# adolliou/euispice_coreg

Measured on AMD Instinct MI355X. Metric: lag-points/sec (whole node) on 2048² grid, 60×60 CRVAL sweep; argmax-shift match, higher is better.
Workload: dtype f64; 1 GPU; headline: Carrington 'fa' 2048x2048 grid lon(200,300) lat(-20,20), 60x60 CRVAL lags arange(-30,30,1) arcsec, small 2048^2 HRIEUV-like, ref 3072^2 FSI-like, order 2, solar_r 1.004; lag_points=3600, parallelism=single GPU, no collective, resident=True, sweeps_in_flight=2, small_stored_f32=True, use_lds=True

## Files before the change

euispice_coreg_amd/csrc/coreg_hip.hip:

```cpp
#include <hip/hip_runtime.h>

#include <algorithm>
#include <chrono>
#include <cmath>
#include <cstdio>
#include <cstdlib>
#include <cstring>
#include <limits>
#include <condition_variable>
#include <map>
#include <memory>
#include <mutex>
#include <string>
#include <thread>
#include <functional>
#include <type_traits>
#include <utility>
#include <vector>

#include "fit.hpp"
#include "geometry.hpp"
#include "kernels.hpp"
#include <atomic>
#include "ricecomp.hpp"
// ... 14 lines not shown
#include "host_sweep_launch.hpp"
#include "host_sweep_mi.hpp"
#include "host_fix_lists.hpp"
#include "host_sweep_io.hpp"
#include "host_context.hpp"
#include "pixels_plan.hpp"
#include "host_pixels.hpp"

coreg_handle::~coreg_handle() = default;

extern "C" {

const char* coreg_version(void) { return "coreg_hip " COREG_VERSION " (gfx950)"; }

int coreg_create(coreg_handle** out, int device) {
    if (!out) return COREG_EINVAL;
    *out = nullptr;
    int ndev = 0;
    hipError_t e = hipGetDeviceCount(&ndev);
    if (e != hipSuccess || ndev < 1) return COREG_EHIP;
    if (device < 0) {
        if (hipGetDevice(&device) != hipSuccess) device = 0;
    }
    if (device >= ndev) return COREG_EINVAL;
    coreg_handle* h = new (std::nothrow) coreg_handle();
    if (!h) return COREG_ENOMEM;
    h->device = device;
    if (hipSetDevice(device) != hipSuccess || hipStreamCreateWithFlags(&h->stream.s, hipStreamNonBlocking) != hipSuccess ||
        hipEventCreate(&h->ev_end[0].e) != hipSuccess ||
        hipEventCreate(&h->ev_end[1].e) != hipSuccess || hipEventRecord(h->ev_end[0], h->stream) != hipSuccess ||
        hipEventRecord(h->ev_end[1], h->stream) != hipSuccess ||
        h->pivots.reserve(2 * sizeof(double)) != hipSuccess ||
        hipMemsetAsync(h->pivots.p, 0, 2 * sizeof(double), h->stream) != hipSuccess) {
        coreg_destroy(h);
        return COREG_EHIP;
    }
    std::memset(&h->stats, 0, sizeof(h->stats));
    *out = h;
    return COREG_OK;
}

void coreg_destroy(coreg_handle* h) {
    if (!h) return;
    (void)hipSetDevice(h->device);
    if (h->up_thread.joinable()) {
        {
            std::unique_lock<std::mutex> lk(h->up_m);
            h->up_cv.wait(lk, [&] { return !h->up_busy && !h->up_has; });
            h->up_stop = true;
        }
        h->up_cv.notify_all();
        h->up_thread.join();
    }
    if (h->stream) (void)hipStreamSynchronize(h->stream);
    if (h->up_stream) (void)hipStreamSynchronize(h->up_stream);
    delete h;
}

const char* coreg_last_error(const coreg_handle* h) { return h ? h->err.c_str() : "null handle"; }

int coreg_set_stream(coreg_handle* h, void* hip_stream) {
    if (!h) return COREG_EINVAL;
    RETCHK(bind_device(h));
    RETCHK(collect_stats(h));
    HIPCHK(hipStreamSynchronize(h->stream));
    HIPCHK(h->stream.borrow((hipStream_t)hip_stream));
    return COREG_OK;
}

int coreg_synchronize(coreg_handle* h) {
    if (!h) return COREG_EINVAL;
    RETCHK(bind_device(h));
    HIPCHK(hipStreamSynchronize(h->stream));
    return COREG_OK;
}

int coreg_set_option(coreg_handle* h, const char* name, int64_t value) {
    if (!h || !name) return COREG_EINVAL;
    const std::string n(name);
    if (n == "use_lds") {
        h->opt_use_lds = value ? 1 : 0;
    } else if (n == "clean_path") {
        h->opt_clean_path = value ? 1 : 0;
    } else if (n == "tap_nan_filter") {
        if (value < 0 || value > 2) return fail(h, COREG_EINVAL, "tap_nan_filter must be 0, 1 or 2");
        h->opt_tap_nan_filter = value;
    } else if (n == "overlap_upload") {
        h->opt_overlap_upload = value ? 1 : 0;
    } else if (n == "async_upload") {
        h->opt_async_upload = value ? 1 : 0;
    } else if (n == "refine") {
        h->opt_refine = value ? 1 : 0;
    } else if (n == "refine_cond_log10") {
        if (value < -3 || value > 15) return fail(h, COREG_EINVAL, "refine_cond_log10 must be in [-3, 15]");
        h->opt_refine_cond_log10 = value;
    } else if (n == "refine_max") {
        if (value < 0 || value > 16) return fail(h, COREG_EINVAL, "refine_max must be in [0, 16]");
    } else if (n == "tile_w") {
        if (value != 0 && (value < 1 || value > kTilePts || (value & (value - 1)) != 0))
            return fail(h, COREG_EINVAL, "tile_w must be 0 or a power of two <= 1024");
        h->opt_tile_w = value;
    } else if (n == "n_groups") {
        if (value < 0) return fail(h, COREG_EINVAL, "n_groups must be >= 0");
        h->opt_n_groups = value;
    } else if (n == "sweep_wgs") {
        if (value < 0) return fail(h, COREG_EINVAL, "sweep_wgs must be >= 0");
        h->opt_sweep_wgs = value;
    } else if (n == "skew") {
        (void)value;
    } else if (n == "shard_world") {
        if (value < 1 || value > 64) return fail(h, COREG_EINVAL, "shard_world must be in [1, 64]");
        h->opt_shard_world = value;
        if (h->opt_shard_rank >= value) h->opt_shard_rank = 0;
    } else if (n == "combo_begin") {
        if (value < 0) return fail(h, COREG_EINVAL, "combo_begin must be >= 0");
        h->opt_combo_begin = value;
    } else if (n == "combo_end") {
        if (value < 0) return fail(h, COREG_EINVAL, "combo_end must be >= 0");
        h->opt_combo_end = value;
    } else if (n == "shard_rank") {
        if (value < 0 || value >= h->opt_shard_world) return fail(h, COREG_EINVAL, "shard_rank must be in [0, shard_world)");
        h->opt_shard_rank = value;
    } else if (n == "border_fix") {
        h->opt_border_fix = value ? 1 : 0;
    } else if (n == "tap_fix") {
        h->opt_tap_fix = value ? 1 : 0;
    } else if (n == "tap_cap") {
        if (value < 1 || value > (1 << 26)) return fail(h, COREG_EINVAL, "tap_cap must be in [1, 2^26]");
        h->opt_tap_cap = value;
    } else if (n == "pitch") {
        h->opt_pitch = value;
    } else if (n == "taper_frac") {
        if (value < -1 || value > 1000) return fail(h, COREG_EINVAL, "taper_frac must be in [-1, 1000]");
        h->opt_taper_frac = value;
    } else if (n == "taper_min") {
        if (value < 16 || value > 1024) return fail(h, COREG_EINVAL, "taper_min must be in [16, 1024]");
        h->opt_taper_min = value;
    } else if (n == "taper_rounds") {
        if (value < 1) return fail(h, COREG_EINVAL, "taper_rounds must be >= 1");
        h->opt_taper_rounds = value;
    } else if (n == "crop_reference") {
        h->opt_crop_reference = value ? 1 : 0;
    } else if (n == "tile_skip") {
        h->opt_tile_skip = value ? 1 : 0;
    } else if (n == "h_series") {
        h->opt_h_series = value ? 1 : 0;
    } else if (n == "h_incr") {
        h->opt_h_incr = value ? 1 : 0;
    } else if (n == "patch_w") {
        if (value < 0 || value > kBlock) return fail(h, COREG_EINVAL, "patch_w must be in [0, 256]");
        h->opt_patch_w = value;
    } else if (n == "mi_chunks") {
        if (value < 0 || value > kMiMaxChunks) return fail(h, COREG_EINVAL, "mi_chunks must be in [0, 64]");
        h->opt_mi_chunks = value;
    } else if (n == "lds_bytes") {
        if (value < 1024 || value > 159 * 1024) return fail(h, COREG_EINVAL, "lds_bytes must be in [1 KiB, 159 KiB]");
        h->opt_lds_bytes = value;
    } else {
        return fail(h, COREG_EINVAL, "unknown option: " + n);
    }
    return COREG_OK;
}

}

#include "abi_images.hpp"
// ... 8 lines not shown
```

euispice_coreg_amd/csrc/host_state.hpp:

```cpp
#pragma once
namespace {

enum SrcKind {
    SRC_HOST = 0,
    SRC_PINNED = 1,
    SRC_DEVICE = 2,
    SRC_TILED = 3,
};

struct PixFmt {
    int bitpix = 0;
    bool f32 = false;
    double bscale = 1.0, bzero = 0.0;
    bool raw() const { return bitpix != 0; }
    bool scaled() const { return bscale != 1.0 || bzero != 0.0; }
    size_t elem() const { return raw() ? (size_t)(bitpix < 0 ? -bitpix : bitpix) / 8 : (f32 ? 4 : 8); }
    bool swap_only() const { return bitpix == -32 && !scaled(); }
    static PixFmt native(bool is_f32) {
        PixFmt f;
        f.f32 = is_f32;
        return f;
    }
};

// ... 45 lines not shown
    int gW = 0, gH = 0;
    int ref_dtype = -1;
    DevBuf pivots, red_sum, red_cnt;
    DevBuf t_sin_lon, t_cos_lon, t_cos_lat, t_sin_lat, t_lon_deg, t_dx;
    coreg_diffrot rot_ref = {}, rot_small = {};
    bool has_rot_ref = false, has_rot_small = false;
    CarrTables tabs;
    std::vector<double> tabs_key;
    bool tabs_uploaded = false;
    PinBuf pin_img[2];
    Event ev_img[2];
    int pin_img_next = 0;
    DevBuf pts, tile_count, tile_list, tile_cum, group_first, tile_info, tile_bbox;
    DevBuf visit_rec;
    DevBuf rf_fix_slab;
    DevBuf counters;
    DevBuf lane_params, out_index, partials, out_dev, tmp_img;
    DevBuf sweep_queue;
    int n_cus = 0;
    struct SweepResidency {
        const void* fn;
        size_t lds_bytes;
        int per_cu;
    };
    std::vector<SweepResidency> sweep_residency;
    int64_t opt_sweep_wgs = 0;
    DevBuf counts;
    long long counts_n = -1;
    DevBuf up_f64, up_flag;
    DevBuf up_raw;
    DevBuf rice_blob, rice_rand, dec_img;
    PrologueArgs pending_prologue = {};
    DevBuf bbox_buf;
    Stream aux_stream;
    Stream up_stream;
    Event ev_small, ev_main;
    bool small_pending = false;
    DevBuf red_sum_up, red_cnt_up;
    int64_t opt_overlap_upload = 1;
    int64_t opt_tap_nan_filter = 2;
    int64_t opt_async_upload = 0;
    std::thread up_thread;
    std::mutex up_m;
    std::condition_variable up_cv;
    std::function<hipError_t()> up_job;
    bool up_has = false, up_stop = false, up_busy = false;
    hipError_t up_rc = hipSuccess;
    PinBuf pin_small[2];
    Event ev_pin_small[2];
    int pin_small_next = 0;
    WcslibCaches wcslib;
    DevBuf border_flags, fix_partial;
    DevBuf border_dev;
    PinBuf pin_border;
    int64_t opt_border_fix = 1;
    int64_t opt_tap_fix = 1, opt_tap_cap = 1 << 24;
    DevBuf tap_count, tap_segq, tap_list, tap_skip, tap_seg_slot, tap_seg_begin, tap_pixel, tap_xw, tap_yw;
    long long tap_last[3] = {0, 0, 0};
    int last_variant[7] = {-1, 0, 0, 0, 0, 0, 0};
    int64_t opt_shard_world = 1, opt_shard_rank = 0;
    int64_t opt_combo_begin = 0, opt_combo_end = 0;
    DevBuf sums;
    long long sums_slots = 0;
    struct PendingFinalize {
        long long slot_off, n_slots, lag_begin;
        int residus;
        RefineArgs refine;
        std::function<int(coreg_handle*)> replay_precompute;
        FixLaunch fixes;
    };
    std::function<int(coreg_handle*)> last_precompute;
    PlanMemo plan_memo;
    DevBuf rf_flags, rf_pivots, rf_list, rf_head, rf_partial;
    std::vector<PendingFinalize> pending_fin;
    DevBuf fin_outidx;
    long long pending_n_out = 0;
    std::vector<double> mi_edges_small, mi_edges_large;
    DevBuf mi_hist;
    size_t mi_lds[6] = {0, 0, 0, 0, 0, 0};
    int64_t opt_mi_chunks = 0;

    int64_t opt_crop_reference = 1;
    int64_t opt_taper_min = 128, opt_taper_frac = -1, opt_taper_rounds = 6;
    int64_t opt_use_lds = 1, opt_clean_path = 1, opt_refine = 1, opt_refine_cond_log10 = 5, opt_tile_w = 0, opt_n_groups = 0, opt_lds_bytes = (159 * 1024 * kPointGroups) / 4, opt_patch_w = 0, opt_h_series = 1, opt_h_incr = 1, opt_tile_skip = 1, opt_pitch = -1;

    coreg_stats stats;
    bool stats_pending = false;
    PinBuf pin_info;
    std::vector<EventPair> ev_sweep, ev_pre;
    size_t ev_sweep_used = 0, ev_pre_used = 0;
    hipEvent_t ev_t1 = nullptr;
    Event ev_end[2];
    PinBuf pin_plan[2];
    int plan_slot = 0;
    bool plan_open = false;
};
```

euispice_coreg_amd/csrc/host_sweep_launch.hpp:

```cpp
#pragma once
namespace {
using sweep_variant::SweepVariant;
static_assert(sweep_variant::kTranslate == MODE_TRANSLATE && sweep_variant::kHomography == MODE_HOMOGRAPHY &&
                  sweep_variant::kHomographySeries == MODE_HOMOGRAPHY_SERIES && sweep_variant::kCar == MODE_CAR &&
                  sweep_variant::kOrderRt == ORDER_RT, "sweep_variant.hpp restates the kernels' constants");

struct SweepLaunchSpec {
    int mode = MODE_TRANSLATE;
    int order = 2;
    int method = COREG_METHOD_CORRELATION;
    size_t slot_off = 0;
    int n_batches = 0, n_tiles = 0;
    long long lag_begin = 0;
    double* out_dev = nullptr;
    const LaunchU* car_inv = nullptr;
    const BorderFix* fix = nullptr;
    int pitch_sel = 0;
    long long n_slots() const { return (long long)n_batches * kBlock; }
    bool residus() const { return method != COREG_METHOD_CORRELATION; }
    int residus_kind() const { return method == COREG_METHOD_RESIDUS_MASKED ? 2 : (residus() ? 1 : 0); }
    const double* params_dev(const coreg_handle* h) const {
        return h->lane_params.as<double>() + (mode == MODE_TRANSLATE ? 2 : 9) * slot_off;
    }
    const long long* outidx_dev(const coreg_handle* h) const { return h->out_index.as<long long>() + slot_off; }
// ... 6 lines not shown
template <size_t... I>
SweepKernel* sweep_kernel_table(std::index_sequence<I...>) {
    constexpr const SweepVariant* v = sweep_variant::kSweepVariants.v;
    static SweepKernel table[] = {
        {k_sweep<v[I].mode, v[I].order, std::conditional_t<v[I].f32, float, double>, v[I].round, v[I].resid, v[I].pitch>, {0}}...};
    return table;
}

int raise_dynamic_lds(coreg_handle* h, SweepKernel* k, size_t lds_bytes) {
    std::lock_guard<std::mutex> lock(g_attr_mutex);
    size_t& ab = k->attr_bytes[h->device % kMaxDevices];
    if (lds_bytes > 48 * 1024 && lds_bytes > ab) {
        HIPCHK(hipFuncSetAttribute((const void*)k->fn, hipFuncAttributeMaxDynamicSharedMemorySize, (int)lds_bytes));
        ab = lds_bytes;
    }
    return COREG_OK;
}

int sweep_grid(coreg_handle* h, const SweepKernel* k, size_t lds_bytes, long long items, unsigned* grid) {
    long long resident = h->opt_sweep_wgs;
    if (resident <= 0) {
        if (h->n_cus <= 0) HIPCHK(hipDeviceGetAttribute(&h->n_cus, hipDeviceAttributeMultiprocessorCount, h->device));
        int per_cu = 0;
        for (const coreg_handle::SweepResidency& r : h->sweep_residency)
            if (r.fn == (const void*)k->fn && r.lds_bytes == lds_bytes) per_cu = r.per_cu;
        if (per_cu <= 0) {
            HIPCHK(hipOccupancyMaxActiveBlocksPerMultiprocessor(&per_cu, (const void*)k->fn, kSweepThreads, lds_bytes));
            if (per_cu <= 0) return fail(h, COREG_EHIP, "launch_sweep: the device holds no k_sweep workgroup of this LDS size");
            h->sweep_residency.push_back({(const void*)k->fn, lds_bytes, per_cu});
        }
        resident = (long long)h->n_cus * per_cu;
    }
    *grid = (unsigned)(8 * ((std::min(items, resident) + 7) / 8));
    return COREG_OK;
}

int launch_k_sweep(coreg_handle* h, const SweepLaunchSpec& L, SweepArgs a, int n_groups8, size_t lds_bytes) {
    const SweepVariant v = sweep_variant::pick_sweep_variant(L.mode, L.order, h->small_f32, L.residus(), L.pitch_sel);
    const int at = sweep_variant::sweep_variant_index(v);
    if (at < 0) return fail(h, COREG_EINVAL, "launch_sweep: no k_sweep instantiation for this mode / order / pitch");
    SweepKernel* k = sweep_kernel_table(std::make_index_sequence<sweep_variant::kNumSweepVariants>()) + at;
    EventPair* ev = next_event(h, h->ev_sweep, h->ev_sweep_used);
    if (!ev) return fail(h, COREG_EHIP, "hipEventCreate failed");
    RETCHK(raise_dynamic_lds(h, k, lds_bytes));
    a.items8 = n_groups8 * L.n_batches;
    unsigned grid = 0;
    RETCHK(sweep_grid(h, k, lds_bytes, 8LL * a.items8, &grid));
    HIPCHK(h->sweep_queue.reserve(8 * sizeof(unsigned)));
    a.queue = h->sweep_queue.as<unsigned>();
    HIPCHK(hipMemsetAsync(a.queue, 0, 8 * sizeof(unsigned), h->stream));
    HIPCHK(hipEventRecord(ev->a, h->stream));
    hipLaunchKernelGGL(k->fn, dim3(grid), dim3(kSweepThreads), lds_bytes, h->stream, a);
    HIPCHK(hipEventRecord(ev->b, h->stream));
    HIPCHK(hipGetLastError());
    const int rec[7] = {at, v.mode, v.order, v.f32 ? 1 : 0, v.round ? 1 : 0, v.resid ? 1 : 0, v.pitch};
    std::copy(rec, rec + 7, h->last_variant);
    return COREG_OK;
}

SweepArgs sweep_args(const coreg_handle* h, const SweepLaunchSpec& L, int n_groups, int group_lo, size_t lds_bytes) {
    SweepArgs a;
    a.img = h->small.p;
    a.W = h->sW;
    a.H = h->sH;
    a.pts = h->pts.as<Pt>();
    a.tile_count = h->tile_count.as<int>();
    a.tile_list = h->tile_list.as<int>();
    a.tile_cum = h->tile_cum.as<int>();
    a.group_first = h->group_first.as<int>();
    a.tile_info = h->tile_info.as<long long>();
    a.tile_bbox = h->tile_bbox.as<double>();
    a.visit_rec = h->visit_rec.as<VisitRec>();
    a.lane_params = L.params_dev(h);
    a.n_slots = L.n_slots();
    a.n_batches = L.n_batches;
    a.n_groups = n_groups;
    a.group_lo = group_lo;
    a.partials = h->partials.as<double>();
    a.queue = nullptr;
    a.items8 = 0;
    a.pivots = h->pivots.as<double>();
    a.use_lds = h->opt_use_lds ? 1 : 0;
    a.clean_path = h->opt_clean_path ? 1 : 0;
    a.lds_elems = (int)(lds_bytes / sizeof(double));
    a.car_inv = L.car_inv ? *L.car_inv : LaunchU{};
    a.car_inv.order_rt = L.order;
    a.car_inv.h_incr = (int)h->opt_h_incr;
    return a;
}

template <typename Args>
void fill_fix_common(Args& x, const coreg_handle* h, const SweepLaunchSpec& L) {
    x.img = h->small.p;
    x.W = h->sW;
    x.H = h->sH;
    x.ref = h->ref.p;
    x.ref_f32 = h->ref_dtype == COREG_F32 ? 1 : 0;
    x.gw = h->gW;
    x.order = L.order;
    x.round_f32 = L.mode == MODE_TRANSLATE ? 0 : 1;
    x.residus = L.residus() ? 1 : 0;
    x.pivots = h->pivots.as<double>();
    x.hom = L.params_dev(h);
    x.n_slots = L.n_slots();
}

int build_fix_launch(coreg_handle* h, const SweepLaunchSpec& L, FixLaunch* fl) {
    fl->small_f32 = h->small_f32;
    if (!L.fix || !L.fix->any()) return COREG_OK;
    static const std::vector<BorderItems::Item> no_items;
    for (const BorderItems::Item& it : L.fix->border ? L.fix->border->items : no_items) {
        if (it.flags_off >= 0) {
            ParityFixArgs p = {};
            fill_fix_common(p, h, L);
            p.flags = h->border_flags.as<unsigned char>() + it.flags_off;
            p.gh = h->gH;
            p.slot = it.slot;
            p.n_partial = 256;
            if (h->fix_partial.reserve((size_t)p.n_partial * kNumSums * sizeof(double)) != hipSuccess)
                return fail(h, COREG_EHIP, "hipMalloc failed (parity fix)");
            p.partial = h->fix_partial.as<double>();
            fl->parity.push_back(p);
        }
        if (it.n == 0) continue;
        BorderFixArgs b = {};
        fill_fix_common(b, h, L);
        b.slot = it.slot;
        b.dropped = h->border_dev.as<int>() + it.first;
        b.n_dropped = it.n;
        fl->border.push_back(b);
    }
    if (L.fix->tap.segs > 0) {
        fl->tap = L.fix->tap;
        fill_fix_common(fl->tap.args, h, L);
    }
    return COREG_OK;
}

int keep_tap_lists(coreg_handle* h, FixLaunch* fixes) {
    auto kept = std::make_shared<KeptTapLists>();
    const size_t nseg = (size_t)fixes->tap.segs, cnt = (size_t)fixes->tap.count;
    TapFixArgs& t = fixes->tap.args;
    const void* src[5] = {t.xw, t.yw, t.pixel, t.seg_begin, t.seg_slot};
    const size_t bytes[5] = {cnt * sizeof(double), cnt * sizeof(double), cnt * sizeof(unsigned), (nseg + 1) * sizeof(int),
                             nseg * sizeof(int)};
    size_t off[6] = {0};
    for (int k = 0; k < 5; ++k) off[k + 1] = off[k] + ((bytes[k] + 7) & ~(size_t)7);
    HIPCHK(kept->all.reserve(off[5]));
    char* all = kept->all.as<char>();
    for (int k = 0; k < 5; ++k)
        if (bytes[k]) HIPCHK(hipMemcpyAsync(all + off[k], src[k], bytes[k], hipMemcpyDeviceToDevice, h->stream));
    t.xw = (const double*)(all + off[0]);
    t.yw = (const double*)(all + off[1]);
    t.pixel = (const unsigned*)(all + off[2]);
    t.seg_begin = (const int*)(all + off[3]);
    t.seg_slot = (const int*)(all + off[4]);
    fixes->kept = kept;
    return COREG_OK;
}

int queue_pending_finalize(coreg_handle* h, const SweepLaunchSpec& L, const RefineArgs& refine, bool refinable,
                           const FixLaunch& fl) {
    coreg_handle::PendingFinalize pf;
    pf.slot_off = (long long)L.slot_off;
    pf.n_slots = L.n_slots();
    pf.lag_begin = L.lag_begin;
// ... 73 lines not shown
```

euispice_coreg_amd/csrc/kernels_sweep.hpp:

```cpp
#pragma once
namespace coreg {
struct SweepArgs {
    const void* img;
    int W, H;
    const Pt* pts;
    const int* tile_count;
    const int* tile_list;
    const int* tile_cum;
    const int* group_first;
    long long* tile_info;
    const double* tile_bbox;
    const VisitRec* visit_rec;
    const double* lane_params;
    long long n_slots;
    int n_batches;
    int n_groups;
    int group_lo;
    double* partials;
    unsigned* queue;
    int items8;
    const double* pivots;
    int use_lds;
    int clean_path;
    int lds_elems;
    LaunchU car_inv;
};

struct Acc {
    int n;
    double a, b, aa, bb, ab;
};

template <int N>
struct Taps;
template <>
struct Taps<3> {
    double t[9];
    __device__ __forceinline__ void issue(unsigned a0, unsigned a1, unsigned a2) {
        asm volatile(
            "ds_read_b64 %0, %9\n\tds_read_b64 %1, %9 offset:8\n\tds_read_b64 %2, %9 offset:16\n\t"
            "ds_read_b64 %3, %10\n\tds_read_b64 %4, %10 offset:8\n\tds_read_b64 %5, %10 offset:16\n\t"
            "ds_read_b64 %6, %11\n\tds_read_b64 %7, %11 offset:8\n\tds_read_b64 %8, %11 offset:16"
            : "=&v"(t[0]), "=&v"(t[1]), "=&v"(t[2]), "=&v"(t[3]), "=&v"(t[4]), "=&v"(t[5]), "=&v"(t[6]), "=&v"(t[7]),
              "=&v"(t[8])
            : "v"(a0), "v"(a1), "v"(a2));
    }
    __device__ __forceinline__ void wait_after(double& w0, double& w1, double& w2) {
        asm volatile("s_waitcnt lgkmcnt(0)"
                     : "+v"(t[0]), "+v"(t[1]), "+v"(t[2]), "+v"(t[3]), "+v"(t[4]), "+v"(t[5]), "+v"(t[6]), "+v"(t[7]),
                       "+v"(t[8]), "+v"(w0), "+v"(w1), "+v"(w2));
    }
    __device__ __forceinline__ void issue_before(unsigned a0, unsigned a1, unsigned a2, double& fx, double& fy) {
        asm volatile(
            "ds_read_b64 %0, %11\n\tds_read_b64 %1, %11 offset:8\n\tds_read_b64 %2, %11 offset:16\n\t"
            "ds_read_b64 %3, %12\n\tds_read_b64 %4, %12 offset:8\n\tds_read_b64 %5, %12 offset:16\n\t"
            "ds_read_b64 %6, %13\n\tds_read_b64 %7, %13 offset:8\n\tds_read_b64 %8, %13 offset:16"
            : "=&v"(t[0]), "=&v"(t[1]), "=&v"(t[2]), "=&v"(t[3]), "=&v"(t[4]), "=&v"(t[5]), "=&v"(t[6]), "=&v"(t[7]),
              "=&v"(t[8]), "+v"(fx), "+v"(fy)
            : "v"(a0), "v"(a1), "v"(a2));
    }
    __device__ __forceinline__ void wait() {
        asm volatile("s_waitcnt lgkmcnt(0)"
                     : "+v"(t[0]), "+v"(t[1]), "+v"(t[2]), "+v"(t[3]), "+v"(t[4]), "+v"(t[5]), "+v"(t[6]), "+v"(t[7]),
                       "+v"(t[8]));
    }
    template <int P>
    __device__ __forceinline__ void issue_before_imm(unsigned a0, double& fx, double& fy) {
        static_assert(P > 0 && (2 * P + 2) * 8 < 65536, "LDS immediate offsets are 16 bits");
        asm volatile(
            "ds_read_b64 %0, %11\n\tds_read_b64 %1, %11 offset:8\n\tds_read_b64 %2, %11 offset:16\n\t"
            "ds_read_b64 %3, %11 offset:%12\n\tds_read_b64 %4, %11 offset:%13\n\tds_read_b64 %5, %11 offset:%14\n\t"
            "ds_read_b64 %6, %11 offset:%15\n\tds_read_b64 %7, %11 offset:%16\n\tds_read_b64 %8, %11 offset:%17"
            : "=&v"(t[0]), "=&v"(t[1]), "=&v"(t[2]), "=&v"(t[3]), "=&v"(t[4]), "=&v"(t[5]), "=&v"(t[6]), "=&v"(t[7]),
              "=&v"(t[8]), "+v"(fx), "+v"(fy)
            : "v"(a0), "n"(P * 8), "n"(P * 8 + 8), "n"(P * 8 + 16), "n"(2 * P * 8), "n"(2 * P * 8 + 8),
              "n"(2 * P * 8 + 16));
    }
};
template <>
struct Taps<2> {
    double t[4];
    __device__ __forceinline__ void issue(unsigned a0, unsigned a1, unsigned) {
        asm volatile(
            "ds_read_b64 %0, %4\n\tds_read_b64 %1, %4 offset:8\n\t"
            "ds_read_b64 %2, %5\n\tds_read_b64 %3, %5 offset:8"
            : "=&v"(t[0]), "=&v"(t[1]), "=&v"(t[2]), "=&v"(t[3])
            : "v"(a0), "v"(a1));
    }
    __device__ __forceinline__ void issue_before(unsigned a0, unsigned a1, unsigned a2, double&, double&) {
        issue(a0, a1, a2);
    }
    __device__ __forceinline__ void wait() {
        asm volatile("s_waitcnt lgkmcnt(0)" : "+v"(t[0]), "+v"(t[1]), "+v"(t[2]), "+v"(t[3]));
    }
};

template <>
struct Taps<4> {
    double t[16];
    __device__ __forceinline__ void issue_before(unsigned a0, unsigned a1, unsigned a2, unsigned a3, double& fx,
                                                 double& fy) {
        asm volatile(
            "ds_read_b64 %0, %18\n\tds_read_b64 %1, %18 offset:8\n\tds_read_b64 %2, %18 offset:16\n\t"
            "ds_read_b64 %3, %18 offset:24\n\t"
            "ds_read_b64 %4, %19\n\tds_read_b64 %5, %19 offset:8\n\tds_read_b64 %6, %19 offset:16\n\t"
            "ds_read_b64 %7, %19 offset:24\n\t"
// ... 449 lines not shown
                            ux = xn * r;
                            uy = yn * r;
                        }
                        point_lag<MODE, ORDER, TS, LDS, ROUND, RESID, INTERIOR, PITCH, CLEAN, true>(
                            acc, win, img, pitch, ox, oy, W, H, wmax, hmax, px0, py0, pxw, pyw, hv, cu, ux, uy,
                            spt_f64(cur, 2), spt_f64(cur, 3), pivot_b);
                        if constexpr (CLEAN) {
                            if (k == 1) acc.a += spt_f64(cur, 3);
                            if (k == 2) acc.aa += spt_f64(cur, 3);
                            if (k == kChunk - 1) acc.n += kChunk;
                        }
                        spt_wait(nxt);
                        cur = nxt;
                    }
                }
            }
            if (pg == n_full % kPointGroups) {
                for (int p = n_full * kChunk; p < p_end; ++p) {
                    Pt pt;
                    load_pt_uniform(pts + p, pt);
                    point_lag<MODE, ORDER, TS, LDS, ROUND, RESID, INTERIOR, PITCH>(acc, win, img, pitch, ox, oy, W, H, wmax,
                                                                                   hmax, px0, py0, pxw, pyw, hm, cu, pt.b0,
                                                                                   pt.b1, pt.a, pt.pad, pivot_b);
                }
            }
            return;
        }
    }
    {
        int c = p_begin / kChunk + pg;
        if (c < n_full) {
            H9 hml = hm;
            double& anchor = MODE == MODE_TRANSLATE ? (INTERIOR && LDS ? pxw : px0) : hml.h[MODE == MODE_CAR ? 0 : 7];
            SPt cur = spt_load(pts + c * kChunk, anchor);
            spt_wait(cur);
            for (; c < n_full; c += kPointGroups) {
                const Pt* __restrict__ q = pts + c * kChunk;
#pragma unroll
                for (int k = 0; k < kChunk; ++k) {
                    SPt nxt = spt_load(k + 1 < kChunk ? q + k + 1 : q + kPointGroups * kChunk, anchor);
                    point_lag<MODE, ORDER, TS, LDS, ROUND, RESID, INTERIOR, PITCH, CLEAN>(
                        acc, win, img, pitch, ox, oy, W, H, wmax, hmax, px0, py0, pxw, pyw, hml, cu, spt_f64(cur, 0),
                        spt_f64(cur, 1), spt_f64(cur, 2), spt_f64(cur, 3), pivot_b);
                    if constexpr (CLEAN) {
                        if (k == 1) acc.a += spt_f64(cur, 3);
                        if (k == 2) acc.aa += spt_f64(cur, 3);
                        if (k == kChunk - 1) acc.n += kChunk;
                    }
                    spt_wait(nxt);
                    cur = nxt;
                }
            }
        }
    }
#else
    for (int c = p_begin / kChunk + pg; c < n_full; c += kPointGroups) {
        const Pt* __restrict__ q = pts + c * kChunk;
        Pt pt[kChunk];
#pragma unroll
        for (int k = 0; k < kChunk; ++k) load_pt_uniform(q + k, pt[k]);
#pragma unroll
        for (int k = 0; k < kChunk; ++k)
            point_lag<MODE, ORDER, TS, LDS, ROUND, RESID, INTERIOR, PITCH, CLEAN>(acc, win, img, pitch, ox, oy, W, H, wmax,
                                                                                  hmax, px0, py0, pxw, pyw, hm, cu, pt[k].b0,
                                                                                  pt[k].b1, pt[k].a, pt[k].pad, pivot_b);
        if constexpr (CLEAN) {
            acc.n += kChunk;
            acc.a += pt[1].pad;
            acc.aa += pt[2].pad;
        }
    }
#endif
    if (pg == n_full % kPointGroups) {
        for (int p = n_full * kChunk; p < p_end; ++p) {
            Pt pt;
            load_pt_uniform(pts + p, pt);
            point_lag<MODE, ORDER, TS, LDS, ROUND, RESID, INTERIOR, PITCH>(acc, win, img, pitch, ox, oy, W, H, wmax, hmax,
                                                                           px0, py0, pxw, pyw, hm, cu, pt.b0, pt.b1, pt.a,
                                                                           pt.pad, pivot_b);
        }
    }
}

template <int MODE, int ORDER, typename TS, bool ROUND, bool RESID, int PITCH = 0>
__global__ void __launch_bounds__(kSweepThreads) k_sweep(const SweepArgs a) {
    extern __shared__ __align__(16) unsigned char lds_raw[];
    double* lds = (double*)lds_raw;
    constexpr int kWaves = kSweepThreads / 64;
    constexpr int kLagWaves = kBlock / 64;
    __shared__ double wred2[2][kLagWaves][4];
    __shared__ int wdirty[2][kWaves];
    constexpr bool kCleanPath = MODE != MODE_CAR && !RESID && ORDER != ORDER_RT && !(ROUND && sizeof(TS) == 8);
    int n_vis = 0, n_vis_lds = 0, n_vis_int = 0, n_vis_clean = 0;

    __shared__ int next_q[2];
    const int slot8 = blockIdx.x & 7;
    int q = blockIdx.x >> 3;
    int item_par = 0;

    const int lane = threadIdx.x & 63, wave = threadIdx.x >> 6;
    const int pg = __builtin_amdgcn_readfirstlane(wave % kPointGroups);
    const int lw = __builtin_amdgcn_readfirstlane(wave / kPointGroups);
    const int ls = 64 * lw + lane;

    const TS* __restrict__ img = (const TS*)a.img;
    const int W = a.W, H = a.H;
    const double inf = __builtin_inf();
    const double pivot_b = a.pivots[1];
#if defined(__HIP_DEVICE_COMPILE__)
    const unsigned win = (unsigned)(uintptr_t)(__attribute__((address_space(3))) unsigned char*)lds_raw;
#else
    const unsigned win = 0;
#endif

    while (q < a.items8) {
    const int batch = q % a.n_batches;
    const int group = a.group_lo + (q / a.n_batches) * 8 + slot8;
    const long long slot = (long long)batch * kBlock + ls;
    int visit = 0;

    double px0 = 0.0, py0 = 0.0;
    H9 hm;
#pragma unroll
    for (int k = 0; k < 9; ++k) hm.h[k] = 0.0;
    if (MODE == MODE_TRANSLATE) {
        px0 = a.lane_params[slot];
        py0 = a.lane_params[a.n_slots + slot];
    } else {
#pragma unroll
        for (int k = 0; k < 9; ++k) hm.h[k] = a.lane_params[(long long)k * a.n_slots + slot];
    }

    const bool pad_lane = MODE == MODE_TRANSLATE ? (px0 != px0) : (hm.h[8] != hm.h[8]);

    Acc acc = {0, 0.0, 0.0, 0.0, 0.0, 0.0};

    const int u_lo = a.group_first[1024 + group];
    const int u_hi = a.group_first[1024 + group + 1];

    constexpr bool kLagBox = MODE == MODE_TRANSLATE && COREG_VISIT_LAGBOX;
    double lx0 = 0.0, lx1 = 0.0, ly0 = 0.0, ly1 = 0.0;
    if constexpr (kLagBox) {
        lx0 = lx1 = px0;
        ly0 = ly1 = py0;
        for (int o = 32; o > 0; o >>= 1) {
            lx0 = fmin(lx0, __shfl_xor(lx0, o));
            lx1 = fmax(lx1, __shfl_xor(lx1, o));
            ly0 = fmin(ly0, __shfl_xor(ly0, o));
            ly1 = fmax(ly1, __shfl_xor(ly1, o));
        }
        if (lane == 0 && pg == 0) {
            wred2[0][lw][0] = lx0;
            wred2[0][lw][1] = lx1;
            wred2[0][lw][2] = ly0;
            wred2[0][lw][3] = ly1;
        }
        __syncthreads();
        lx0 = fmin(fmin(wred2[0][0][0], wred2[0][1][0]), fmin(wred2[0][2][0], wred2[0][3][0]));
        lx1 = fmax(fmax(wred2[0][0][1], wred2[0][1][1]), fmax(wred2[0][2][1], wred2[0][3][1]));
        ly0 = fmin(fmin(wred2[0][0][2], wred2[0][1][2]), fmin(wred2[0][2][2], wred2[0][3][2]));
        ly1 = fmax(fmax(wred2[0][0][3], wred2[0][1][3]), fmax(wred2[0][2][3], wred2[0][3][3]));
    }

    int tl = a.group_first[group];
    unsigned park = 0;
    {
        Visit first;
        load_visit_uniform(a.visit_rec + tl, first);
        park = park_visit(first, park);
    }
    for (; u_lo < u_hi; ++tl) {
        Visit cur;
        unpark_visit(park, cur);
        const int ubase = cur.ubase;
        if (ubase >= u_hi) break;
        Visit nxt;
        load_visit_uniform(a.visit_rec + tl + 1, nxt);
        const int tile = cur.tile;
        const int cnt = cur.cnt;
        const int p_begin = max(u_lo - ubase, 0) * kUnitPts;
        const int p_end = min((u_hi - ubase) * kUnitPts, cnt);
        if (p_begin >= p_end) {
            park = park_visit(nxt, park);
            continue;
        }
        const double bx0 = cur.bx0, bx1 = cur.bx1, by0 = cur.by0, by1 = cur.by1;

        double mnx, mxx, mny, mxy;
        if constexpr (kLagBox) {
            mnx = bx0 + lx0;
            mxx = bx1 + lx1;
            mny = by0 + ly0;
            mxy = by1 + ly1;
        } else if (MODE == MODE_TRANSLATE) {
            mnx = bx0 + px0;
            mxx = bx1 + px0;
            mny = by0 + py0;
            mxy = by1 + py0;
        } else {
            mnx = inf; mxx = -inf; mny = inf; mxy = -inf;
#pragma unroll
            for (int c = 0; c < 4; ++c) {
                double cx, cy;
                apply_map<MODE>(hm, a.car_inv, (c & 1) ? bx1 : bx0, (c & 2) ? by1 : by0, cx, cy);
                mnx = fmin(mnx, cx);
                mxx = fmax(mxx, cx);
                mny = fmin(mny, cy);
                mxy = fmax(mxy, cy);
            }
            if (MODE == MODE_CAR) {
                const double margin = car_tile_margin(a.car_inv.box_c, fmax(fabs(by0), fabs(by1)) + a.car_inv.pole_sep);
                mnx -= margin;
                mxx += margin;
                mny -= margin;
                mxy += margin;
            }
        }
        int* wdirt = wdirty[visit & 1];
        if constexpr (!kLagBox) {
            for (int o = 32; o > 0; o >>= 1) {
                mnx = fmin(mnx, __shfl_xor(mnx, o));
                mxx = fmax(mxx, __shfl_xor(mxx, o));
                mny = fmin(mny, __shfl_xor(mny, o));
                mxy = fmax(mxy, __shfl_xor(mxy, o));
            }
            double(*wred)[4] = wred2[visit & 1];
            if (lane == 0 && pg == 0) {
                wred[lw][0] = mnx;
                wred[lw][1] = mxx;
                wred[lw][2] = mny;
                wred[lw][3] = mxy;
            }
            __syncthreads();
            mnx = fmin(fmin(wred[0][0], wred[1][0]), fmin(wred[2][0], wred[3][0]));
            mxx = fmax(fmax(wred[0][1], wred[1][1]), fmax(wred[2][1], wred[3][1]));
            mny = fmin(fmin(wred[0][2], wred[1][2]), fmin(wred[2][2], wred[3][2]));
            mxy = fmax(fmax(wred[0][3], wred[1][3]), fmax(wred[2][3], wred[3][3]));
        }
        ++visit;
        if (!(mxx >= 0.0) || !(mnx <= (double)(W - 1)) || !(mxy >= 0.0) || !(mny <= (double)(H - 1))) {
            park = park_visit(nxt, park);
            continue;
        }
        if constexpr (kLagBox) __syncthreads();
        constexpr double kClear = 1e-9;
        const bool interior = (mnx >= kClear) & (mxx <= (double)(W - 1) - kClear) & (mny >= kClear) &
                              (mxy <= (double)(H - 1) - kClear);
        constexpr bool kWide = ORDER == ORDER_RT || ORDER > 2;
        const int ord = ORDER == ORDER_RT ? a.car_inv.order_rt : ORDER;
        const int ap_lo = kWide ? ord / 2 + 1 : 1;
        const int ap_hi = kWide ? ord - ord / 2 + 1 : 2;
        const int ox = max((int)floor(fmax(mnx, 0.0)) - ap_lo, kWide ? -ap_lo : -1);
        const int oy = max((int)floor(fmax(mny, 0.0)) - ap_lo, kWide ? -ap_lo : -1);
        const int ex = min((int)floor(fmin(mxx, (double)(W - 1))) + ap_hi, kWide ? W - 1 + ap_hi : W);
        const int ey = min((int)floor(fmin(mxy, (double)(H - 1))) + ap_hi, kWide ? H - 1 + ap_hi : H);
        const int ww = ex - ox + 1, wh = ey - oy + 1;
        int pitch = PITCH > 0 ? PITCH : (ww | 1);
        if (PITCH == 0) {
            const int r = pitch & 31;
            const int up = r < 5 ? 5 - r : ((r > 11 && r < 21) ? 21 - r : (r > 27 ? 37 - r : 0));
            if ((long long)(pitch + up) * wh <= (long long)a.lds_elems) pitch += up;
        }
        const long long need = (long long)pitch * wh;
        const bool in_lds = a.use_lds && (need <= (long long)a.lds_elems) && (PITCH == 0 || ww <= PITCH);

        const Pt* __restrict__ pts = a.pts + (size_t)tile * kTilePts;

        bool swept = false;
        ++n_vis;
        {
          if (in_lds) {
            swept = true;
            ++n_vis_lds;
#ifndef COREG_STAGE_ROWS
#define COREG_STAGE_ROWS 8
#endif
#ifndef COREG_STAGE_COLS
#define COREG_STAGE_COLS 1
#endif
            constexpr int kStage = COREG_STAGE_ROWS, kCols = COREG_STAGE_COLS;
            const double scale = ORDER == 2 ? 0.25 : 1.0;
            constexpr bool kFmaStage = ORDER == 2 && !ROUND && COREG_VISIT_FMA;
            const double npivot4 = -0.25 * pivot_b;
            const int wave_u = __builtin_amdgcn_readfirstlane(wave);
            double poison = 0.0;
            for (int r0 = wave_u; r0 < wh; r0 += kWaves * kStage) {
                for (int c0 = 0; c0 < ww; c0 += 64 * kCols) {
                    int gx[kCols];
#pragma unroll
                    for (int j = 0; j < kCols; ++j) {
                        const int c = c0 + 64 * j + lane;
                        gx[j] = kWide ? mirror_far(ox + min(c, ww - 1), W) : mirror_idx(ox + min(c, ww - 1), W);
                    }
                    TS v[kStage][kCols];
#pragma unroll
                    for (int k = 0; k < kStage; ++k) {
                        const int r = min(r0 + k * kWaves, wh - 1);
                        const int gy = kWide ? mirror_far(oy + r, H) : mirror_idx(oy + r, H);
                        const TS* __restrict__ row = img + (size_t)gy * W;
#pragma unroll
                        for (int j = 0; j < kCols; ++j) v[k][j] = row[gx[j]];
                    }
#pragma unroll
                    for (int j = 0; j < kCols; ++j) {
                        const int c = c0 + 64 * j + lane;
                        if (c < ww) {
#pragma unroll
                            for (int k = 0; k < kStage; ++k) {
                                const int r = r0 + k * kWaves;
                                if (r < wh) {
                                    const double e = (kFmaStage ? fma((double)v[k][j], 0.25, npivot4)
                                                                : (ROUND ? (double)v[k][j] : (double)v[k][j] - pivot_b) * scale);
                                    lds[r * pitch + c] = e;
                                    if (kCleanPath) poison = fma(e, 0.0, poison);
                                }
                            }
                        }
                    }
                }
            }
            park = park_visit(nxt, park);
            if (kCleanPath && interior) {
                const int dirty = __ballot(poison != poison) != 0ull;
                if (lane == 0) wdirt[wave] = dirty;
            }
            __syncthreads();
            bool done = false;
            if constexpr (ORDER != ORDER_RT) {
                if (interior) {
                    done = true;
                    bool clean = false;
                    if constexpr (kCleanPath) clean = a.clean_path && __ballot(wdirt[lane % kWaves] != 0) == 0ull;
                    ++n_vis_int;
                    n_vis_clean += clean ? 1 : 0;
                    if (!pad_lane) {
                        const double offx = (ORDER == 2 ? 0.5 : 0.0) - (double)(ORDER / 2 + ox);
                        const double offy = (ORDER == 2 ? 0.5 : 0.0) - (double)(ORDER / 2 + oy);
                        const double pxw = MODE == MODE_TRANSLATE ? px0 + offx : offx;
                        const double pyw = MODE == MODE_TRANSLATE ? py0 + offy : offy;
                        if (kCleanPath && clean) {
                            tile_points<MODE, ORDER, TS, true, ROUND, RESID, true, PITCH, kCleanPath>(
                                acc, win, img, pitch, ox, oy, W, H, px0, py0, pxw, pyw, hm, a.car_inv, pts, p_begin, p_end,
                                pivot_b, pg);
                        } else {
                            tile_points<MODE, ORDER, TS, true, ROUND, RESID, true, PITCH>(acc, win, img, pitch, ox, oy, W, H,
                                                                                          px0, py0, pxw, pyw, hm, a.car_inv,
                                                                                          pts, p_begin, p_end, pivot_b, pg);
                        }
                    }
                }
            }
            if (!done) {
                const double offx = ORDER == 2 ? 0.5 - (double)(1 + ox) : (ORDER == 3 ? -(double)(1 + ox) : 0.0);
                const double offy = ORDER == 2 ? 0.5 - (double)(1 + oy) : (ORDER == 3 ? -(double)(1 + oy) : 0.0);
                tile_points<MODE, ORDER, TS, true, ROUND, RESID, false, PITCH>(acc, win, img, pitch, ox, oy, W, H, px0, py0,
                                                                               offx, offy, hm, a.car_inv, pts, p_begin,
                                                                               p_end, pivot_b, pg);
            }
          }
        }
        if (!swept) {
            park = park_visit(nxt, park);
            tile_points<MODE, ORDER, TS, false, ROUND, RESID>(acc, win, img, 0, 0, 0, W, H, px0, py0, 0.0, 0.0, hm, a.car_inv, pts,
                                                              p_begin, p_end, pivot_b, pg);
        }
    }

    unsigned ticket = 0;
    if (threadIdx.x == 0) ticket = atomicAdd(a.queue + slot8, 1u);
    __syncthreads();
    if (threadIdx.x == 0) next_q[item_par] = (int)(gridDim.x >> 3) + (int)ticket;
    if (pg > 0) {
        double* st = lds + ((size_t)(pg - 1) * kNumSums) * kBlock + ls;
        st[0] = (double)acc.n;
        st[kBlock] = acc.a;
        st[2 * kBlock] = acc.b;
        st[3 * kBlock] = acc.aa;
        st[4 * kBlock] = acc.bb;
        st[5 * kBlock] = acc.ab;
    }
    __syncthreads();
    if (pg == 0) {
        double sn = (double)acc.n, sa = acc.a, sb = acc.b, saa = acc.aa, sbb = acc.bb, sab = acc.ab;
        for (int g = 0; g < kPointGroups - 1; ++g) {
            const double* st = lds + ((size_t)g * kNumSums) * kBlock + ls;
            sn += st[0];
            sa += st[kBlock];
            sb += st[2 * kBlock];
            saa += st[3 * kBlock];
            sbb += st[4 * kBlock];
            sab += st[5 * kBlock];
        }
        double* out = a.partials + (size_t)(group - a.group_lo) * kNumSums * a.n_slots + slot;
        out[0] = sn;
        out[a.n_slots] = sa;
        out[2 * a.n_slots] = sb;
        out[3 * a.n_slots] = saa;
        out[4 * a.n_slots] = sbb;
        out[5 * a.n_slots] = sab;
    }
    q = __builtin_amdgcn_readfirstlane(next_q[item_par]);
    item_par ^= 1;
    }

    if (threadIdx.x == 0) {
        atomicAdd((unsigned long long*)a.tile_info + 3, (unsigned long long)n_vis);
        atomicAdd((unsigned long long*)a.tile_info + 4, (unsigned long long)n_vis_lds);
        atomicAdd((unsigned long long*)a.tile_info + 5, (unsigned long long)n_vis_int);
        atomicAdd((unsigned long long*)a.tile_info + 6, (unsigned long long)n_vis_clean);
// ... 5 lines not shown
```

Before: 1.283 million lag-points/s.

## Prefetch next visit's first staging rows into registers during current tile compute

Adds a software-pipelined prefetch. After the LDS staging barrier, each wave computes the next visit's window and loads its first staged row block (two 64-column strips) from global memory into registers. The next visit then writes those registers into LDS instead of reloading them, so global-load latency is hidden behind the current tile's interpolation work. It also adds a straight-line load path that skips mirror indexing when the window lies fully inside the image. The cost is extra registers held across the compute phase, which may lower occupancy, plus a flag carried in a lane of the park register.

```diff
diff --git a/euispice_coreg_amd/csrc/coreg_hip.hip b/euispice_coreg_amd/csrc/coreg_hip.hip
--- a/euispice_coreg_amd/csrc/coreg_hip.hip
+++ b/euispice_coreg_amd/csrc/coreg_hip.hip
@@ -120,6 +120,8 @@
         h->opt_use_lds = value ? 1 : 0;
     } else if (n == "clean_path") {
         h->opt_clean_path = value ? 1 : 0;
+    } else if (n == "visit_prefetch") {
+        h->opt_visit_prefetch = value ? 1 : 0;
     } else if (n == "tap_nan_filter") {
         if (value < 0 || value > 2) return fail(h, COREG_EINVAL, "tap_nan_filter must be 0, 1 or 2");
         h->opt_tap_nan_filter = value;
diff --git a/euispice_coreg_amd/csrc/host_state.hpp b/euispice_coreg_amd/csrc/host_state.hpp
--- a/euispice_coreg_amd/csrc/host_state.hpp
+++ b/euispice_coreg_amd/csrc/host_state.hpp
@@ -151,7 +151,7 @@
 
     int64_t opt_crop_reference = 1;
     int64_t opt_taper_min = 128, opt_taper_frac = -1, opt_taper_rounds = 6;
-    int64_t opt_use_lds = 1, opt_clean_path = 1, opt_refine = 1, opt_refine_cond_log10 = 5, opt_tile_w = 0, opt_n_groups = 0, opt_lds_bytes = (159 * 1024 * kPointGroups) / 4, opt_patch_w = 0, opt_h_series = 1, opt_h_incr = 1, opt_tile_skip = 1, opt_pitch = -1;
+    int64_t opt_use_lds = 1, opt_clean_path = 1, opt_refine = 1, opt_refine_cond_log10 = 5, opt_tile_w = 0, opt_n_groups = 0, opt_lds_bytes = (159 * 1024 * kPointGroups) / 4, opt_patch_w = 0, opt_h_series = 1, opt_h_incr = 1, opt_tile_skip = 1, opt_pitch = -1, opt_visit_prefetch = 1;
 
     coreg_stats stats;
     bool stats_pending = false;
diff --git a/euispice_coreg_amd/csrc/host_sweep_launch.hpp b/euispice_coreg_amd/csrc/host_sweep_launch.hpp
--- a/euispice_coreg_amd/csrc/host_sweep_launch.hpp
+++ b/euispice_coreg_amd/csrc/host_sweep_launch.hpp
@@ -112,6 +112,7 @@
     a.pivots = h->pivots.as<double>();
     a.use_lds = h->opt_use_lds ? 1 : 0;
     a.clean_path = h->opt_clean_path ? 1 : 0;
+    a.visit_prefetch = h->opt_visit_prefetch ? 1 : 0;
     a.lds_elems = (int)(lds_bytes / sizeof(double));
     a.car_inv = L.car_inv ? *L.car_inv : LaunchU{};
     a.car_inv.order_rt = L.order;
diff --git a/euispice_coreg_amd/csrc/kernels_sweep.hpp b/euispice_coreg_amd/csrc/kernels_sweep.hpp
--- a/euispice_coreg_amd/csrc/kernels_sweep.hpp
+++ b/euispice_coreg_amd/csrc/kernels_sweep.hpp
@@ -22,6 +22,7 @@
     const double* pivots;
     int use_lds;
     int clean_path;
+    int visit_prefetch;
     int lds_elems;
     LaunchU car_inv;
 };
@@ -637,6 +638,104 @@
     }
 }
 
+#ifndef COREG_STAGE_ROWS
+#define COREG_STAGE_ROWS 8
+#endif
+#ifndef COREG_STAGE_COLS
+#define COREG_STAGE_COLS 1
+#endif
+#ifndef COREG_PF_COLS
+#define COREG_PF_COLS 2
+#endif
+
+struct VisitWin {
+    bool live, interior, in_lds;
+    bool inside;
+    int ox, oy, ww, wh, pitch;
+};
+template <int ORDER, int PITCH, bool UNIFORM>
+__device__ __forceinline__ VisitWin visit_window(double mnx, double mxx, double mny, double mxy, int W, int H, int order_rt,
+                                                 int use_lds, int lds_elems) {
+    VisitWin w = {false, false, false, false, 0, 0, 0, 0, 0};
+    if (!(mxx >= 0.0) || !(mnx <= (double)(W - 1)) || !(mxy >= 0.0) || !(mny <= (double)(H - 1))) return w;
+    w.live = true;
+    constexpr double kClear = 1e-9;
+    w.interior = (mnx >= kClear) & (mxx <= (double)(W - 1) - kClear) & (mny >= kClear) & (mxy <= (double)(H - 1) - kClear);
+    constexpr bool kWide = ORDER == ORDER_RT || ORDER > 2;
+    const int ord = ORDER == ORDER_RT ? order_rt : ORDER;
+    const int ap_lo = kWide ? ord / 2 + 1 : 1;
+    const int ap_hi = kWide ? ord - ord / 2 + 1 : 2;
+    int ox = max((int)floor(fmax(mnx, 0.0)) - ap_lo, kWide ? -ap_lo : -1);
+    int oy = max((int)floor(fmax(mny, 0.0)) - ap_lo, kWide ? -ap_lo : -1);
+    int ex = min((int)floor(fmin(mxx, (double)(W - 1))) + ap_hi, kWide ? W - 1 + ap_hi : W);
+    int ey = min((int)floor(fmin(mxy, (double)(H - 1))) + ap_hi, kWide ? H - 1 + ap_hi : H);
+    if constexpr (UNIFORM) {
+        ox = __builtin_amdgcn_readfirstlane(ox);
+        oy = __builtin_amdgcn_readfirstlane(oy);
+        ex = __builtin_amdgcn_readfirstlane(ex);
+        ey = __builtin_amdgcn_readfirstlane(ey);
+    }
+    w.ox = ox;
+    w.oy = oy;
+    w.ww = ex - ox + 1;
+    w.wh = ey - oy + 1;
+    w.inside = (ox >= 0) & (oy >= 0) & (ex <= W - 1) & (ey <= H - 1);
+    int pitch = PITCH > 0 ? PITCH : (w.ww | 1);
+    if (PITCH == 0) {
+        const int r = pitch & 31;
+        const int up = r < 5 ? 5 - r : ((r > 11 && r < 21) ? 21 - r : (r > 27 ? 37 - r : 0));
+        if ((long long)(pitch + up) * w.wh <= (long long)lds_elems) pitch += up;
+    }
+    w.pitch = pitch;
+    const long long need = (long long)pitch * w.wh;
+    w.in_lds = use_lds && (need <= (long long)lds_elems) && (PITCH == 0 || w.ww <= PITCH);
+    return w;
+}
+
+constexpr int kStageWaves = kSweepThreads / 64;
+template <int ORDER, bool STRAIGHT, typename TS, int N>
+__device__ __forceinline__ void stage_load(TS (&v)[N], const TS* __restrict__ img, int W, int H, const VisitWin& w, int r0,
+                                           int c0, int lane) {
+    constexpr bool kWide = ORDER == ORDER_RT || ORDER > 2;
+    const int c = w.ox + min(c0 + lane, w.ww - 1);
+    if (STRAIGHT && w.inside) {
+#pragma unroll
+        for (int k = 0; k < N; ++k) {
+            const TS* __restrict__ row = img + (size_t)(w.oy + min(r0 + k * kStageWaves, w.wh - 1)) * W;
+            v[k] = row[c];
+        }
+    } else {
+        const int gx = kWide ? mirror_far(c, W) : mirror_idx(c, W);
+#pragma unroll
+        for (int k = 0; k < N; ++k) {
+            const int r = min(r0 + k * kStageWaves, w.wh - 1);
+            const int gy = kWide ? mirror_far(w.oy + r, H) : mirror_idx(w.oy + r, H);
+            const TS* __restrict__ row = img + (size_t)gy * W;
+            v[k] = row[gx];
+        }
+    }
+}
+template <int ORDER, bool ROUND, bool POISON, typename TS, int N>
+__device__ __forceinline__ void stage_store(const TS (&v)[N], double* __restrict__ lds, const VisitWin& w, int r0, int c0,
+                                            int lane, double pivot_b, double& poison) {
+    const double scale = ORDER == 2 ? 0.25 : 1.0;
+    constexpr bool kFmaStage = ORDER == 2 && !ROUND && COREG_VISIT_FMA;
+    const double npivot4 = -0.25 * pivot_b;
+    const int c = c0 + lane;
+    if (c < w.ww) {
+#pragma unroll
+        for (int k = 0; k < N; ++k) {
+            const int r = r0 + k * kStageWaves;
+            if (r < w.wh) {
+                const double e = (kFmaStage ? fma((double)v[k], 0.25, npivot4)
+                                            : (ROUND ? (double)v[k] : (double)v[k] - pivot_b) * scale);
+                lds[r * w.pitch + c] = e;
+                if (POISON) poison = fma(e, 0.0, poison);
+            }
+        }
+    }
+}
+
 template <int MODE, int ORDER, typename TS, bool ROUND, bool RESID, int PITCH = 0>
 __global__ void __launch_bounds__(kSweepThreads) k_sweep(const SweepArgs a) {
     extern __shared__ __align__(16) unsigned char lds_raw[];
@@ -647,6 +746,14 @@
     __shared__ int wdirty[2][kWaves];
     constexpr bool kCleanPath = MODE != MODE_CAR && !RESID && ORDER != ORDER_RT && !(ROUND && sizeof(TS) == 8);
     int n_vis = 0, n_vis_lds = 0, n_vis_int = 0, n_vis_clean = 0;
+    constexpr int kPfCols = COREG_PF_COLS;
+    constexpr bool kPrefetch = MODE == MODE_TRANSLATE && COREG_VISIT_LAGBOX && ORDER == 2 && sizeof(TS) == 4 && !ROUND &&
+                               !RESID && COREG_STAGE_COLS == 1 && kPfCols > 0;
+    TS pf[kPrefetch ? kPfCols : 1][COREG_STAGE_ROWS];
+#pragma unroll
+    for (int j = 0; j < (kPrefetch ? kPfCols : 1); ++j)
+#pragma unroll
+        for (int k = 0; k < COREG_STAGE_ROWS; ++k) pf[j][k] = (TS)0;
 
     __shared__ int next_q[2];
     const int slot8 = blockIdx.x & 7;
@@ -727,6 +834,11 @@
     for (; u_lo < u_hi; ++tl) {
         Visit cur;
         unpark_visit(park, cur);
+        bool from_regs = false;
+        if constexpr (kPrefetch) {
+            from_regs = __builtin_amdgcn_readlane((int)park, 11) != 0;
+            write_lane<11>(park, 0u);
+        }
         const int ubase = cur.ubase;
         if (ubase >= u_hi) break;
         Visit nxt;
@@ -793,31 +905,15 @@
             mxy = fmax(fmax(wred[0][3], wred[1][3]), fmax(wred[2][3], wred[3][3]));
         }
         ++visit;
-        if (!(mxx >= 0.0) || !(mnx <= (double)(W - 1)) || !(mxy >= 0.0) || !(mny <= (double)(H - 1))) {
+        const VisitWin vw = visit_window<ORDER, PITCH, kPrefetch>(mnx, mxx, mny, mxy, W, H, a.car_inv.order_rt, a.use_lds,
+                                                                   a.lds_elems);
+        if (!vw.live) {
             park = park_visit(nxt, park);
             continue;
         }
         if constexpr (kLagBox) __syncthreads();
-        constexpr double kClear = 1e-9;
-        const bool interior = (mnx >= kClear) & (mxx <= (double)(W - 1) - kClear) & (mny >= kClear) &
-                              (mxy <= (double)(H - 1) - kClear);
-        constexpr bool kWide = ORDER == ORDER_RT || ORDER > 2;
-        const int ord = ORDER == ORDER_RT ? a.car_inv.order_rt : ORDER;
-        const int ap_lo = kWide ? ord / 2 + 1 : 1;
-        const int ap_hi = kWide ? ord - ord / 2 + 1 : 2;
-        const int ox = max((int)floor(fmax(mnx, 0.0)) - ap_lo, kWide ? -ap_lo : -1);
-        const int oy = max((int)floor(fmax(mny, 0.0)) - ap_lo, kWide ? -ap_lo : -1);
-        const int ex = min((int)floor(fmin(mxx, (double)(W - 1))) + ap_hi, kWide ? W - 1 + ap_hi : W);
-        const int ey = min((int)floor(fmin(mxy, (double)(H - 1))) + ap_hi, kWide ? H - 1 + ap_hi : H);
-        const int ww = ex - ox + 1, wh = ey - oy + 1;
-        int pitch = PITCH > 0 ? PITCH : (ww | 1);
-        if (PITCH == 0) {
-            const int r = pitch & 31;
-            const int up = r < 5 ? 5 - r : ((r > 11 && r < 21) ? 21 - r : (r > 27 ? 37 - r : 0));
-            if ((long long)(pitch + up) * wh <= (long long)a.lds_elems) pitch += up;
-        }
-        const long long need = (long long)pitch * wh;
-        const bool in_lds = a.use_lds && (need <= (long long)a.lds_elems) && (PITCH == 0 || ww <= PITCH);
+        const bool interior = vw.interior, in_lds = vw.in_lds;
+        const int ox = vw.ox, oy = vw.oy, ww = vw.ww, wh = vw.wh, pitch = vw.pitch;
 
         const Pt* __restrict__ pts = a.pts + (size_t)tile * kTilePts;
 
@@ -827,51 +923,34 @@
           if (in_lds) {
             swept = true;
             ++n_vis_lds;
-#ifndef COREG_STAGE_ROWS
-#define COREG_STAGE_ROWS 8
-#endif
-#ifndef COREG_STAGE_COLS
-#define COREG_STAGE_COLS 1
-#endif
             constexpr int kStage = COREG_STAGE_ROWS, kCols = COREG_STAGE_COLS;
-            const double scale = ORDER == 2 ? 0.25 : 1.0;
-            constexpr bool kFmaStage = ORDER == 2 && !ROUND && COREG_VISIT_FMA;
-            const double npivot4 = -0.25 * pivot_b;
             const int wave_u = __builtin_amdgcn_readfirstlane(wave);
             double poison = 0.0;
-            for (int r0 = wave_u; r0 < wh; r0 += kWaves * kStage) {
-                for (int c0 = 0; c0 < ww; c0 += 64 * kCols) {
-                    int gx[kCols];
-#pragma unroll
-                    for (int j = 0; j < kCols; ++j) {
-                        const int c = c0 + 64 * j + lane;
-                        gx[j] = kWide ? mirror_far(ox + min(c, ww - 1), W) : mirror_idx(ox + min(c, ww - 1), W);
-                    }
-                    TS v[kStage][kCols];
-#pragma unroll
-                    for (int k = 0; k < kStage; ++k) {
-                        const int r = min(r0 + k * kWaves, wh - 1);
-                        const int gy = kWide ? mirror_far(oy + r, H) : mirror_idx(oy + r, H);
-                        const TS* __restrict__ row = img + (size_t)gy * W;
-#pragma unroll
-                        for (int j = 0; j < kCols; ++j) v[k][j] = row[gx[j]];
-                    }
-#pragma unroll
-                    for (int j = 0; j < kCols; ++j) {
-                        const int c = c0 + 64 * j + lane;
-                        if (c < ww) {
-#pragma unroll
-                            for (int k = 0; k < kStage; ++k) {
-                                const int r = r0 + k * kWaves;
-                                if (r < wh) {
-                                    const double e = (kFmaStage ? fma((double)v[k][j], 0.25, npivot4)
-                                                                : (ROUND ? (double)v[k][j] : (double)v[k][j] - pivot_b) * scale);
-                                    lds[r * pitch + c] = e;
-                                    if (kCleanPath) poison = fma(e, 0.0, poison);
-                                }
-                            }
+            int r0 = wave_u;
+            if constexpr (kPrefetch) {
+                if (from_regs) {
+                    if (r0 < wh) {
+#pragma unroll
+                        for (int j = 0; j < kPfCols; ++j)
+                            if (64 * j < ww)
+                                stage_store<ORDER, ROUND, kCleanPath>(pf[j], lds, vw, r0, 64 * j, lane, pivot_b, poison);
+                        for (int c0 = 64 * kPfCols; c0 < ww; c0 += 64) {
+                            TS v[kStage];
+                            stage_load<ORDER, kPrefetch>(v, img, W, H, vw, r0, c0, lane);
+                            stage_store<ORDER, ROUND, kCleanPath>(v, lds, vw, r0, c0, lane, pivot_b, poison);
                         }
                     }
+                    r0 += kWaves * kStage;
+                }
+            }
+            for (; r0 < wh; r0 += kWaves * kStage) {
+                for (int c0 = 0; c0 < ww; c0 += 64 * kCols) {
+                    TS v[kCols][kStage];
+#pragma unroll
+                    for (int j = 0; j < kCols; ++j) stage_load<ORDER, kPrefetch>(v[j], img, W, H, vw, r0, c0 + 64 * j, lane);
+#pragma unroll
+                    for (int j = 0; j < kCols; ++j)
+                        stage_store<ORDER, ROUND, kCleanPath>(v[j], lds, vw, r0, c0 + 64 * j, lane, pivot_b, poison);
                 }
             }
             park = park_visit(nxt, park);
@@ -879,7 +958,29 @@
                 const int dirty = __ballot(poison != poison) != 0ull;
                 if (lane == 0) wdirt[wave] = dirty;
             }
+            if constexpr (kPrefetch) __builtin_amdgcn_s_waitcnt(0x0F70);
             __syncthreads();
+            if constexpr (kPrefetch) {
+                if (a.visit_prefetch) {
+                    Visit nv;
+                    unpark_visit(park, nv);
+                    const int nb = max(u_lo - nv.ubase, 0) * kUnitPts;
+                    const int ne = min((u_hi - nv.ubase) * kUnitPts, nv.cnt);
+                    if (nv.ubase < u_hi && nb < ne) {
+                        const VisitWin nw = visit_window<ORDER, PITCH, kPrefetch>(nv.bx0 + lx0, nv.bx1 + lx1, nv.by0 + ly0,
+                                                                                   nv.by1 + ly1, W, H, a.car_inv.order_rt,
+                                                                                   a.use_lds, a.lds_elems);
+                        if (nw.live && nw.in_lds) {
+                            if (wave_u < nw.wh) {
+#pragma unroll
+                                for (int j = 0; j < kPfCols; ++j)
+                                    if (64 * j < nw.ww) stage_load<ORDER, kPrefetch>(pf[j], img, W, H, nw, wave_u, 64 * j, lane);
+                            }
+                            write_lane<11>(park, 1u);
+                        }
+                    }
+                }
+            }
             bool done = false;
             if constexpr (ORDER != ORDER_RT) {
                 if (interior) {
```

New measurement: 1.262 million lag-points/s. 0.984x the previous value.
